# jl6017/AutoURDF

Hardware: AMD Instinct MI355X
Metric: registered frames/sec (N=4096 pts, K=20 clusters) (higher is better)
Workload: dtype f32

## Files before the change

### autourdf_amd/csrc/train_backward.hip

```cpp
#include <cmath>
#include <cstddef>
#include <cstring>
#include "train_dev.h"

namespace creg {

__device__ __forceinline__ TrainState advance_state(const TrainState& S, float loss, const Hyper& hy, double bc1, float bc2_sqrt) {
    TrainState N = S;
    const bool improved = loss < S.min_loss;
    N.last_loss = loss;
    N.epochs_run = S.epochs_run + 1;
    const int count = improved ? 0 : S.count + 1;
    N.min_loss = improved ? loss : S.min_loss;
    N.best_epoch = improved ? S.epochs_run : S.best_epoch;
    N.count = count;
    N.stopped = (!improved && count > hy.stop) ? 1 : S.stopped;
    if (!N.stopped) {
        N.step = S.step + 1;
        N.step_size = (float)(S.lr / bc1);
        N.bc2_sqrt = bc2_sqrt;
        const double cur = (double)loss;
        if (cur < S.sched_best * (1.0 - 1e-4)) { N.sched_best = cur; N.sched_bad = 0; }
        else N.sched_bad = S.sched_bad + 1;
        if (N.sched_bad > hy.patience) {
            const double nl = fmax(S.lr * (double)hy.factor, 0.0);
            if (S.lr - nl > 1e-8) N.lr = nl;
            N.sched_bad = 0;
        }
    }
    return N;
}

constexpr int GC_QMAX = 3;
__device__ __forceinline__ void gradc_role(const Dims& D, const Ws& W, int epoch, int nbx, int nby, int k) {
    __shared__ float red[4][14];
    __shared__ float s_loss;
    __shared__ float s_go[16];
    const int tid = threadIdx.x, lane = tid & 63, wv = tid >> 6;
    const TrainState S = W.state[epoch & 1];
    const int b0 = W.off[k], e0 = W.off[k + 1];
    const Hyper hy = *W.hyper;
    float a = tid < nbx ? W.lossp_x[tid] : 0.f, b = tid < nby ? W.lossp_y[tid] : 0.f;
    const float m2v = W.m2[16 * k + (tid & 15)];
    float sv[16];
#pragma unroll
    for (int i = 0; i < 16; ++i) sv[i] = W.head_save[16 * k + i];
    const float* h2cur = (epoch & 1) ? W.h2[1] : W.h2[0];
    float w3v[GC_QMAX][8], h2v[GC_QMAX];
#pragma unroll
    for (int q = 0; q < GC_QMAX; ++q) {
        const int o = min(q * 256 + tid, D.H2 - 1);
        const bool isA = o < D.HA;
        const float* Pc = (epoch & 1) ? W.P1 : W.P;
        const float* wb = isA ? Pc + D.oW3A + o : Pc + D.oW3B + (o - D.HA);
        const int stride = isA ? D.HA : D.HB, nj = isA ? D.OA : D.OB;
#pragma unroll
        for (int j = 0; j < 8; ++j) w3v[q][j] = wb[(size_t)min(j, nj - 1) * stride];
        h2v[q] = h2cur[(size_t)k * D.H2 + o];
    }
    asm volatile("" :: "v"(a), "v"(b), "v"(m2v), "v"(sv[0]), "v"(sv[1]), "v"(sv[2]), "v"(sv[3]), "v"(sv[4]), "v"(sv[5]), "v"(sv[6]), "v"(sv[7]),
                 "v"(sv[8]), "v"(sv[9]), "v"(sv[10]), "v"(sv[11]), "v"(sv[12]), "v"(sv[13]), "v"(sv[14]), "v"(sv[15]), "v"(b0), "v"(e0), "v"(hy.lr));
#pragma unroll
    for (int q = 0; q < GC_QMAX; ++q)
        asm volatile("" :: "v"(h2v[q]), "v"(w3v[q][0]), "v"(w3v[q][1]), "v"(w3v[q][2]), "v"(w3v[q][3]), "v"(w3v[q][4]), "v"(w3v[q][5]), "v"(w3v[q][6]),
                     "v"(w3v[q][7]));
    if (S.stopped) {
        if (k == 0 && tid == 0) {
            TrainState E = S; E.stopped = 1;
            W.state[(epoch + 1) & 1] = E;
        }
        return;
    }
    const int n_first = min(b0 + tid, D.NP - 1);
    const float4 p_first = W.pts4[n_first];
    const int4 c_first = W.cnt4[n_first];
    const int s_first = W.sgn_x[n_first];
    const float4 pr_first = W.pred4[n_first];
    for (int i = tid + 256; i < nbx; i += 256) a += W.lossp_x[i];
    for (int i = tid + 256; i < nby; i += 256) b += W.lossp_y[i];
    a = wave_sum_fast(a); b = wave_sum_fast(b);
    if (lane == 0) { red[wv][0] = a; red[wv][1] = b; }
    __syncthreads();
    if (tid == 0) {
        const float sa = ((red[0][0] + red[1][0]) + red[2][0]) + red[3][0];
        const float sb = ((red[0][1] + red[1][1]) + red[2][1]) + red[3][1];
        s_loss = sa / (float)D.NP + sb / (float)D.NT;
    }
    __syncthreads();
    const float loss = s_loss;
    TrainState N = advance_state(S, loss, hy, S.next_bc1, S.next_bc2s);
    const bool improved = loss < S.min_loss;
    if (improved) {
        for (int n = b0 + tid; n < e0; n += 256) {
            const float4 p = (n == b0 + tid) ? pr_first : W.pred4[n];
            W.best_pred[3 * (size_t)n] = p.x; W.best_pred[3 * (size_t)n + 1] = p.y; W.best_pred[3 * (size_t)n + 2] = p.z;
        }
        if (tid < 16) W.best_m[16 * k + tid] = m2v;
    }
    if (k == 0 && tid == 0) {
        N.next_bc1 = W.bc1[min(N.step + 1, D.epochs)];
        N.next_bc2s = W.bc2s[min(N.step + 1, D.epochs)];
        W.state[(epoch + 1) & 1] = N;
        W.loss_hist[S.epochs_run] = loss;
        W.lr_hist[S.epochs_run] = (float)S.lr;
        W.result[0] = N.min_loss; W.result[1] = (float)N.epochs_run; W.result[2] = (float)N.lr; W.result[3] = (float)N.best_epoch;
    }
    if (N.stopped) return;
    const float gx = 1.0f / (float)D.NP, gy = 1.0f / (float)D.NT;
    float acc[12];
#pragma unroll
    for (int i = 0; i < 12; ++i) acc[i] = 0.f;
    for (int n = b0 + tid; n < e0; n += 256) {
        const bool first = n == b0 + tid;
        const float4 p = first ? p_first : W.pts4[n];
        const int4 c = first ? c_first : W.cnt4[n];
        const int sb = first ? s_first : W.sgn_x[n];
        const float g[3] = {((sb & 1) ? gx : -gx) + gy * (float)c.x, ((sb & 2) ? gx : -gx) + gy * (float)c.y,
                            ((sb & 4) ? gx : -gx) + gy * (float)c.z};
#pragma unroll
        for (int q = 0; q < 3; ++q) {
            acc[4 * q] = fmaf(g[q], p.x, acc[4 * q]); acc[4 * q + 1] = fmaf(g[q], p.y, acc[4 * q + 1]);
            acc[4 * q + 2] = fmaf(g[q], p.z, acc[4 * q + 2]); acc[4 * q + 3] += g[q];
        }
    }
    __syncthreads();
#pragma unroll
    for (int i = 0; i < 12; ++i) { const float r = wave_sum_fast(acc[i]); if (lane == 0) red[wv][i] = r; }
    __syncthreads();
    if (tid == 0) {
        float G12[12];
        for (int i = 0; i < 12; ++i) G12[i] = ((red[0][i] + red[1][i]) + red[2][i]) + red[3][i];
        for (int i = 0; i < 16; ++i) W.gm2[16 * k + i] = i < 12 ? G12[i] : 0.f;
        const float G[9] = {G12[0], G12[1], G12[2], G12[4], G12[5], G12[6], G12[8], G12[9], G12[10]};
        const float gt[3] = {G12[3], G12[7], G12[11]};
        float go[16];
        for (int i = 0; i < 16; ++i) go[i] = 0.f;
        if (D.rot == ROT_6D) {
            go[0] = gt[0]; go[1] = gt[1]; go[2] = gt[2];
            rot6d_to_matrix_vjp(sv, G, go + 4);
        } else if (D.rot == ROT_RPY) {
            go[0] = gt[0]; go[1] = gt[1]; go[2] = gt[2];
            float ge[3];
            euler_xyz_to_matrix_vjp(sv, G, ge);
            for (int i = 0; i < 3; ++i) go[4 + i] = ge[i] * (1.f - sv[4 + i] * sv[4 + i]);
        } else if (D.rot == ROT_Q) {
            go[0] = gt[0]; go[1] = gt[1]; go[2] = gt[2];
            float gu[4];
            quat_to_matrix_vjp(sv, G, gu);
            const float nrm = sv[4];
            if (nrm > 1e-12f) {
                const float dot = sv[0] * gu[0] + sv[1] * gu[1] + sv[2] * gu[2] + sv[3] * gu[3];
#pragma unroll
                for (int i = 0; i < 4; ++i) go[4 + i] = (gu[i] - sv[i] * dot) / nrm;
            } else {
#pragma unroll
                for (int i = 0; i < 4; ++i) go[4 + i] = gu[i] / 1e-12f;
            }
        } else {
            float gdq[8];
            dq_to_se3_vjp(sv, G, gt, gdq);
            for (int i = 0; i < 8; ++i) go[4 + i] = gdq[i];
        }
        for (int i = 0; i < 12; ++i) { W.g_out[16 * k + i] = go[i]; s_go[i] = go[i]; }
    }
    __syncthreads();
#pragma unroll
    for (int q = 0; q < GC_QMAX; ++q) {
        const int o = q * 256 + tid;
        if (o < D.H2) {
            const bool isA = o < D.HA;
            const int nj = isA ? D.OA : D.OB, gofs = isA ? 0 : 4;
            float sum = 0.f;
#pragma unroll
            for (int j = 0; j < 8; ++j) if (j < nj) sum = fmaf(s_go[gofs + j], w3v[q][j], sum);
            W.g_h2[(size_t)k * D.H2 + o] = sum * act_grad(h2v[q], D.slope);
        }
    }
}

__global__ __launch_bounds__(256) void k_gradc(Dims D, Ws W0, int epoch, int nbx, int nby, size_t bstride) {
    asm volatile("" :: "s"(W0.P), "s"(W0.P1), "s"(W0.h2[0]), "s"(W0.h2[1]), "s"(W0.head_save), "s"(W0.m2), "s"(W0.gm2), "s"(W0.pts4), "s"(W0.pred4),
                 "s"(W0.sgn_x), "s"(W0.cnt4), "s"(W0.lossp_x), "s"(W0.lossp_y), "s"(W0.g_out), "s"(W0.g_h2), "s"(W0.state), "s"(W0.bc1), "s"(W0.bc2s),
                 "s"(W0.best_m), "s"(W0.best_pred), "s"(W0.loss_hist), "s"(W0.lr_hist), "s"(W0.result), "s"(W0.off), "s"(W0.hyper),
                 "s"(D.rot), "s"(D.K), "s"(D.H2), "s"(D.HA), "s"(D.HB), "s"(D.OA), "s"(D.OB), "s"(D.NP), "s"(D.NT), "s"(D.epochs), "s"(D.slope),
                 "s"(D.oW3A), "s"(D.oW3B), "s"(epoch), "s"(nbx), "s"(nby), "s"(bstride));
    const Ws W = ws_shift(W0, blockIdx.z * bstride);
    gradc_role(D, W, epoch, nbx, nby, blockIdx.x);
}

__device__ __forceinline__ float adam_value(float p, float& mm, float& vv, float g, float step_size, float bc2_sqrt) {
    const float b1w = (float)(1.0 - 0.9), b2 = 0.999f, b2w = (float)(1.0 - 0.999);
    mm = mm + b1w * (g - mm);
    vv = vv * b2 + (b2w * g) * g;
    const float denom = sqrtf(vv) / bc2_sqrt + 1e-8f;
    return p + (-step_size * mm) / denom;
}

#ifdef CREG_BD_STAMPS
struct BdStamps {
    unsigned long long first[256], endB[256], endD[256], startB[256], startD[256];
    unsigned long long phase[2][8], blocks[2];
    int armed;
};
__device__ BdStamps g_bd_st;
#endif
constexpr int BD_THREADS = 512;
constexpr int B2_THREADS = BD_THREADS;
constexpr int B2_WAVES = B2_THREADS / 64;
constexpr int B2_CB = 16;
constexpr int B2_RB = 32;
__host__ __device__ inline int b2_smem_floats(int K, int IN, int H2) {
    return B2_WAVES * B2_RB * B2_CB + K * IN + 2 * K * B2_CB + H2 * B2_CB;
}
__device__ __forceinline__ float row_sum16(float v) {
    CREG_DPP_STEP(v, 0xB1, 0xF);
    CREG_DPP_STEP(v, 0x4E, 0xF);
    CREG_DPP_STEP(v, 0x141, 0xF);
    CREG_DPP_STEP(v, 0x140, 0xF);
    return v;
}

template <int KW, bool X>
__device__ __forceinline__ void bwd2_role(const Dims& D, const Ws& W, int epoch, int blk, float* sh, unsigned long long bd_entry) {
    constexpr int NS = KW / 4;
    constexpr bool V4 = KW % 16 == 0;
    constexpr int NA = V4 ? NS / 4 : NS;
    float* red = sh;
    float* encs = red + B2_WAVES * B2_RB * B2_CB;
    float* gxs = encs + D.K * D.IN;
    float* xt = gxs + D.K * B2_CB;
    float* w2s = xt + D.K * B2_CB;
    const int tid = threadIdx.x, lane = tid & 63, wv = tid >> 6, lj = lane & 15, kk = lane >> 4;
    __builtin_amdgcn_s_waitcnt(0x0F70);
    const int c0 = blk * B2_CB, par = epoch & 1;
    const float* x1cur = par ? W.x1[1] : W.x1[0];
    float* x1next = par ? W.x1[0] : W.x1[1];
    const float* Pc = par ? W.P1 : W.P;
    float* Pn = par ? W.P : W.P1;
    BD_T0
    {
        const float* src = Pc + D.oW2 + (size_t)(wv * KW + (lane >> 2)) * D.H + c0 + 4 * (lane & 3);
        float* dst = w2s + wv * KW * B2_CB;
#pragma unroll
        for (int i = 0; i < KW; i += 16)
            if (i + (lane >> 2) < KW)
                __builtin_amdgcn_global_load_lds((const __attribute__((address_space(1))) void*)(src + (size_t)i * D.H),
                                                 (__attribute__((address_space(3))) void*)(dst + i * B2_CB), 16, 0, 0);
    }
    const float* gbase = W.g_h2 + wv * KW + (V4 ? 4 * kk : kk);
    auto load_a = [&](int row, float* dst) {
        const float* g = gbase + (size_t)min(row, D.K - 1) * D.H2;
#pragma unroll
        for (int q = 0; q < NA; ++q) {
            if constexpr (V4) { const float4 v = *(const float4*)(g + 16 * q); dst[4 * q] = v.x; dst[4 * q + 1] = v.y; dst[4 * q + 2] = v.z; dst[4 * q + 3] = v.w; }
            else dst[q] = g[4 * q];
        }
    };
    float a0[NS], a1[NS];
    const bool two0 = D.K > 16;
    load_a(lj, a0);
    if (two0) load_a(16 + lj, a1);
    const int half = tid >> 8, t2 = tid & 255, row = t2 >> 4, i4 = t2 & 15, hu = c0 + row;
    const bool ain = 4 * i4 < D.IN;
    const int ei = min(4 * i4, D.IN - 4);
    const size_t wi = (size_t)D.oW1 + (size_t)hu * D.IN + ei;
    float4 pw = *(const float4*)(Pc + wi), pm = *(const float4*)(W.AM + wi), pv = *(const float4*)(W.AV + wi);
    const bool ain2 = X && 64 + 4 * i4 < D.IN;
    const int ei2 = min(64 + 4 * i4, D.IN - 4);
    const size_t wi2 = (size_t)D.oW1 + (size_t)hu * D.IN + ei2;
    float4 pw2, pm2, pv2;
// ... 313 lines not shown
```

### autourdf_amd/csrc/train_dev.h

```cpp
#pragma once
#include <type_traits>
#include "creg_common.h"
#include "creg_dev.h"

namespace creg {

struct Dims {
    int rot, K, KP, IN, H, HA, HB, H2, OA, OB, NP, NT, epochs;
    float slope;
    int oW1, ob1, oW2, ob2, oW3A, ob3A, oW3B, ob3B, NPAR;
    int nbx, nby;
    int nyb;
    int npb;
    int ppl;
    int nbt, nbp;
    int rows;
};

constexpr int PS_MAXB = 512;
constexpr int YS_CHUNK = 16384;

struct Hyper {
    float lr, factor;
    int patience, stop;
};

struct TrainState {
    double lr, sched_best;
    int sched_bad, count, stopped, step;
    float min_loss;
    int epochs_run, best_epoch;
    float step_size, bc2_sqrt;
    float last_loss;
    float next_bc2s;
    double next_bc1;
};

struct Ws {
    float *P, *P1, *AM, *AV;
    float *pose_in, *enc, *x1[2], *h2[2], *head_save, *m2, *gm2;
    float4 *pts4, *y4, *pred4, *ys4, *psl4, *ps4;
    float *ybox, *pbox;
    int* sb;
    int* sgn_x;
    int4* cnt4;
    float *lossp_x, *lossp_y;
    float *g_out, *g_h2;
    TrainState* state;
    double* bc1;
    float* bc2s;
    float *best_m, *best_pred, *loss_hist, *lr_hist, *result;
    int* off;
    Hyper* hyper;
    unsigned long long* ysum;
};

static_assert(sizeof(Ws) % sizeof(char*) == 0, "Ws must hold pointers only");
__host__ __device__ __forceinline__ Ws ws_shift(Ws W, size_t bytes) {
    char** p = reinterpret_cast<char**>(&W);
#pragma unroll
    for (size_t i = 0; i < sizeof(Ws) / sizeof(char*); ++i) p[i] += bytes;
    return W;
}

constexpr int ROT_Q = 0, ROT_DQ = 1, ROT_6D = 2, ROT_RPY = 3;
constexpr int POSE_IN = 12;
typedef float f32x4 __attribute__((ext_vector_type(4)));
typedef float nn_f2 __attribute__((ext_vector_type(2)));
__device__ __forceinline__ float act_f(float v, float slope) { return v > 0.f ? v : v * slope; }
__device__ __forceinline__ float act_grad(float post, float slope) { return post > 0.f ? 1.f : slope; }

__device__ __forceinline__ int seg_of(const int* __restrict__ off, int k, int n) {
    int lo = 0, hi = k;
    while (hi - lo > 1) { const int mid = (lo + hi) >> 1; if (off[mid] <= n) lo = mid; else hi = mid; }
    return lo;
}

#ifdef CREG_BD_STAMPS
#define BD_T0 unsigned long long bd_t[8]; int bd_n = 0; if (threadIdx.x == 0) bd_t[bd_n++] = bd_entry;
#define BD_T  if (threadIdx.x == 0) bd_t[bd_n++] = wall_clock64();
#define BD_TEND(role, epoch) do { asm volatile("s_waitcnt vmcnt(0)" ::: "memory"); if (threadIdx.x == 0) { bd_t[bd_n++] = wall_clock64(); \
    if (g_bd_st.armed) { const int sl_ = (epoch) & 255; atomicMin(&g_bd_st.first[sl_], bd_t[0]); \
        atomicMin(role ? &g_bd_st.startD[sl_] : &g_bd_st.startB[sl_], bd_t[0]); atomicMax(role ? &g_bd_st.endD[sl_] : &g_bd_st.endB[sl_], bd_t[bd_n - 1]); \
        for (int k_ = 1; k_ < bd_n; ++k_) atomicAdd(&g_bd_st.phase[role][k_ - 1], bd_t[k_] - bd_t[k_ - 1]); atomicAdd(&g_bd_st.blocks[role], 1ull); } } } while (0)
#else
#define BD_T0
#define BD_T
#define BD_TEND(role, epoch)
#endif

constexpr int BATCH_MAX = 64;
struct Slice { Ws W; int nz; };

template <int V, int... Vs, typename F>
static void by_value(int v, F f) {
    if constexpr (sizeof...(Vs) == 0) f(std::integral_constant<int, V>{});
    else if (v == V) f(std::integral_constant<int, V>{});
    else by_value<Vs...>(v, f);
}
template <typename F>
static void by_nc(int H, F f) { by_value<1, 2, 4, 8>(H / 64, f); }

struct ParamMap { int off, count; };
int param_map(const Dims& D, ParamMap* pm);
constexpr int COPY_MAX = 150;
struct CopyTable { const unsigned* src[COPY_MAX]; unsigned* dst[COPY_MAX]; int n[COPY_MAX]; int count = 0; };
void copy_table_add(CopyTable& T, const void* src, void* dst, size_t bytes, hipStream_t s);
void copy_table_launch(CopyTable& T, hipStream_t s);
int setup_raise_lds(const Dims& D);
int stage_inputs(const Dims& D, const Slice& S, size_t bstride, const creg_train_args* args, hipStream_t s);
void launch_sorts(const Dims& D, const Slice& S, size_t bstride, hipStream_t s, bool keep_target_blocks);
void launch_params_home(const Dims& D, const Slice& S, size_t bstride, int sidx, int step0, hipStream_t s);
void launch_set_state(const Dims& D, const Ws& W, const creg_train_state& from, hipStream_t s);
void launch_get_state(const Ws& W, int sidx, double* out, hipStream_t s);
void launch_l2(const Dims& D, const Slice& S, size_t bstride, int par, hipStream_t s);
void launch_head(const Dims& D, const Slice& S, size_t bstride, int par, hipStream_t s);
void launch_nn(const Dims& D, const Slice& S, size_t bstride, int par, hipStream_t s);
bool backward_fits(const Dims& D);
int bd_raise_lds(const Dims& D);
void launch_gradc(const Dims& D, const Slice& S, size_t bstride, int epoch, hipStream_t s);
void launch_bd(const Dims& D, const Slice& S, size_t bstride, int epoch, hipStream_t s);
int bd_stamps_arm(bool on);

}
```

### autourdf_amd/csrc/train_engine.hip

```cpp
#include <chrono>
#include <cstdlib>
#include <cstring>
#include <memory>
#include <vector>
#include "train_dev.h"
#include "nn_l1.h"

namespace creg {

constexpr int CHAINS_MAX = 8;

struct Plan {
    creg_train_shape shape{};
    Dims D{};
    Ws W{};
    ParamMap pm[10] = {};
    int np = 0;
    int B = 1;
    size_t bstride = 0;
    int branches = 1;
    hipGraphExec_t gexec = nullptr;
    bool graph_ready = false;
    int graph_epochs = 0;
    bool chain_streams = false;
// ... 176 lines not shown

static int pick_chain_streams(Plan* P, hipStream_t s) {
    static const bool probe = !(getenv("CREG_NO_QUEUE_PROBE") && getenv("CREG_NO_QUEUE_PROBE")[0] == '1');
    constexpr int ATTEMPTS = 7;
    P->probe_us = 0;
    auto fits = [](double t) { return t >= 0 && t < SPIN_TOGETHER_US; };
    auto accept = [&](double t) { if (P->probe_us >= 0 && (int)t > P->probe_us) P->probe_us = (int)t; };
    for (int gi = 1; gi < P->branches; ++gi) {
        hipStream_t set[CHAINS_MAX + 1], rejected[ATTEMPTS + 1];
        int ns = 0, nr = 0;
        set[ns++] = s;
        for (int j = 1; j < gi; ++j) set[ns++] = P->cst[j];
        hipStream_t chosen = nullptr;
        if (P->cst[gi]) {
            set[ns] = P->cst[gi];
            const double t = candidate_spin_us(set, ns + 1);
            if (!probe || fits(t)) { chosen = P->cst[gi]; if (probe) accept(t); }
            else { (void)hipStreamSynchronize(P->cst[gi]); rejected[nr++] = P->cst[gi]; P->cst[gi] = nullptr; }
        }
        for (int attempt = 0; !chosen && attempt < ATTEMPTS; ++attempt) {
            hipStream_t cs = nullptr;
            if (hipStreamCreateWithFlags(&cs, hipStreamNonBlocking) != hipSuccess) break;
            if (!probe) { chosen = cs; break; }
            set[ns] = cs;
            const double t = candidate_spin_us(set, ns + 1);
            if (fits(t)) { chosen = cs; accept(t); }
            else rejected[nr++] = cs;
        }
        if (!chosen && nr) { chosen = rejected[--nr]; P->probe_us = -1; }
        for (int i = 0; i < nr; ++i) (void)hipStreamDestroy(rejected[i]);
        if (!chosen) {
            (void)hipGetLastError();
            creg::set_error("creg_train_plan_run_batch: cannot create a stream for chain %d", gi);
            return CREG_EHIP;
        }
        P->cst[gi] = chosen;
    }
    P->cal_stream = s; P->cal_done = true;
    return CREG_OK;
}

static int capture_chains(Plan* P, int epg) {
    FirstError fe;
    if (!P->cfork) CREG_TRY(fe, hipEventCreateWithFlags(&P->cfork, hipEventDisableTiming));
    ScopedStream cs;
    CREG_TRY(fe, hipStreamCreateWithFlags(&cs.h, hipStreamNonBlocking));
    for (int gi = 0; gi < P->branches && fe.ok(); ++gi) {
        ScopedGraph g;
        if (gi > 0 && !P->cjoin[gi]) CREG_TRY(fe, hipEventCreateWithFlags(&P->cjoin[gi], hipEventDisableTiming));
        if (P->cexec[gi]) { (void)hipGraphExecDestroy(P->cexec[gi]); P->cexec[gi] = nullptr; }
        CREG_TRY(fe, hipStreamBeginCapture(cs.h, hipStreamCaptureModeThreadLocal));
        if (fe.ok()) {
            const Slice S = chain_slice(P, gi);
            for (int i = 0; i < epg; ++i) enqueue_epoch(P, S, i, cs.h);
            fe.note(hipStreamEndCapture(cs.h, &g.h), "hipStreamEndCapture");
        }
        CREG_TRY(fe, hipGraphInstantiate(&P->cexec[gi], g.h, nullptr, nullptr, 0));
    }
    if (!fe.ok()) {
        (void)hipGetLastError();
        for (int gi = 0; gi < CHAINS_MAX; ++gi) if (P->cexec[gi]) { (void)hipGraphExecDestroy(P->cexec[gi]); P->cexec[gi] = nullptr; }
        creg::set_error("creg_train_plan_run_batch: chain graph capture failed: %s: %s", fe.what, hipGetErrorString(fe.err));
        return CREG_EHIP;
    }
    P->graph_ready = true;
    P->graph_epochs = epg;
    return CREG_OK;
}

static int run_chains(Plan* P, hipStream_t s) {
    const Dims& D = P->D;
    if (P->branches > 1 && (!P->cal_done || P->cal_stream != s))
        if (int rc = pick_chain_streams(P, s)) return rc;
    auto st_of = [&](int gi) { return gi == 0 ? s : P->cst[gi]; };
    FirstError fe;
    CREG_TRY(fe, hipEventRecord(P->cfork, s));
    for (int gi = 1; gi < P->branches; ++gi) CREG_TRY(fe, hipStreamWaitEvent(P->cst[gi], P->cfork, 0));
    int e = 0;
    for (; fe.ok() && e + P->graph_epochs <= D.epochs; e += P->graph_epochs)
        for (int gi = 0; gi < P->branches; ++gi) CREG_TRY(fe, hipGraphLaunch(P->cexec[gi], st_of(gi)));
    for (int gi = 0; fe.ok() && gi < P->branches; ++gi) {
        const Slice S = chain_slice(P, gi);
        for (int e2 = e; e2 < D.epochs; ++e2) enqueue_epoch(P, S, e2, st_of(gi));
    }
    for (int gi = 1; gi < P->branches; ++gi) {
        if (hipEventRecord(P->cjoin[gi], P->cst[gi]) != hipSuccess || hipStreamWaitEvent(s, P->cjoin[gi], 0) != hipSuccess) {
            (void)hipStreamSynchronize(P->cst[gi]);
            fe.note(hipErrorUnknown, "joining a chain stream");
        }
    }
    if (!fe.ok()) {
        (void)hipGetLastError();
        creg::set_error("creg_train_plan_run_batch: %s: %s", fe.what, hipGetErrorString(fe.err));
        return CREG_EHIP;
    }
    return CREG_OK;
}

static int begin_run(const char* who, Plan* P, const Slice& S, const creg_train_args* args, bool with_outputs, bool may_keep_leaves,
                     hipStream_t s) {
    bool keep = may_keep_leaves && P->target_blocks_valid;
    for (int b = 0; b < S.nz; ++b) {
        const creg_train_args* a = args + b;
        CREG_REQUIRE(a->m && a->y && a->local_pts && a->seg_offsets && a->params && (!with_outputs || (a->best_m && a->best_pred && a->result)),
                     "%s: null pointer in problem %d", who, b);
        for (int i = 0; i < P->np; ++i) CREG_REQUIRE(a->params[i], "%s: params[%d] of problem %d is null", who, i, b);
        keep = keep && a->y_unchanged != 0;
    }
    if (int rc = stage_inputs(P->D, S, P->bstride, args, s)) return rc;
    launch_sorts(P->D, S, P->bstride, s, keep);
    P->target_blocks_valid = may_keep_leaves;
    return CREG_OK;
}

static void results_out(const Plan* P, const Slice& S, const creg_train_args* args, CopyTable& T, hipStream_t s) {
    const Dims& D = P->D;
    for (int b = 0; b < S.nz; ++b) {
        const creg_train_args* a = args + b;
        const Ws W = ws_shift(S.W, (size_t)b * P->bstride);
        for (int i = 0; i < P->np; ++i) copy_table_add(T, W.P + P->pm[i].off, a->params[i], sizeof(float) * P->pm[i].count, s);
        copy_table_add(T, W.best_m, a->best_m, sizeof(float) * 16 * D.K, s);
        copy_table_add(T, W.best_pred, a->best_pred, sizeof(float) * 3 * D.NP, s);
        copy_table_add(T, W.result, a->result, sizeof(float) * 4, s);
        if (a->loss_hist) copy_table_add(T, W.loss_hist, a->loss_hist, sizeof(float) * D.epochs, s);
        if (a->lr_hist) copy_table_add(T, W.lr_hist, a->lr_hist, sizeof(float) * D.epochs, s);
    }
    copy_table_launch(T, s);
}

static int batch_of(const creg_train_shape* s) { return s->batch >= 1 ? s->batch : 1; }

extern "C" size_t creg_train_workspace_bytes(const creg_train_shape* shape) {
    Dims D;
    if (!make_dims(shape, &D) || shape->batch < 0 || shape->batch > BATCH_MAX) return 0;
    return align_up(carve(D, nullptr, nullptr), 256) * batch_of(shape);
}

extern "C" int creg_train_plan_create(const creg_train_shape* shape, void* workspace, size_t workspace_bytes,
                                      creg_train_plan** plan) {
    Dims D;
    CREG_REQUIRE(plan && workspace, "creg_train_plan_create: null pointer");
    CREG_REQUIRE(make_dims(shape, &D), "creg_train_plan_create: unsupported shape (rot in 0..3, hidden in {64, 128, 256, 512}, 1 <= k <= 256 with the K x IN features + the B role's tiles inside 160 KB of LDS, sizes >= 1)");
    CREG_REQUIRE(((uintptr_t)workspace & 255) == 0, "creg_train_plan_create: workspace must be 256-byte aligned");
    CREG_REQUIRE(shape->batch >= 0 && shape->batch <= BATCH_MAX, "creg_train_plan_create: batch must be in [0, %d]", BATCH_MAX);
    const size_t one = align_up(carve(D, nullptr, nullptr), 256), need = one * batch_of(shape);
    CREG_REQUIRE(workspace_bytes >= need, "creg_train_plan_create: workspace too small (%zu < %zu)", workspace_bytes, need);
    auto P = std::make_unique<Plan>();
    P->shape = *shape; P->D = D; P->np = param_map(D, P->pm);
    carve(D, (char*)workspace, &P->W);
    P->B = batch_of(shape); P->bstride = one;
    const int auto_chains = (D.NT > 64 * 64 && P->B >= 3) ? 3 : (P->B >= 8 ? 3 : (P->B >= 5 ? 2 : 1));
    P->chain_streams = shape->graph_branches <= 0;
    P->branches = shape->graph_branches > 0 ? shape->graph_branches : (shape->graph_branches < 0 ? -shape->graph_branches : auto_chains);
    if (P->branches > P->B) P->branches = P->B;
    if (P->branches > CHAINS_MAX) P->branches = CHAINS_MAX;
    if (int rc = bd_raise_lds(D)) return rc;
    if (int rc = setup_raise_lds(D)) return rc;
    *plan = (creg_train_plan*)P.release();
    return CREG_OK;
}

extern "C" int creg_train_plan_run_batch(creg_train_plan* plan, const creg_train_args* args, int32_t n,
                                         creg_stream_t stream) {
    Plan* P = (Plan*)plan;
    CREG_REQUIRE(P && args, "creg_train_plan_run_batch: null pointer");
    CREG_REQUIRE(n == P->B, "creg_train_plan_run_batch: the plan was created for a batch of %d problems, got %d", P->B, n);
    hipStream_t s = (hipStream_t)stream;
    const Dims& D = P->D;
    const Slice all = slice_of(P, 0, P->B);
    if (int rc = begin_run("creg_train_plan_run_batch", P, all, args, true, true, s)) return rc;
    int e = 0;
    if (P->shape.use_graph && D.epochs >= 2) {
        int epg = P->shape.use_graph > 1 ? P->shape.use_graph : 50;
        if (epg > D.epochs) epg = D.epochs;
        epg &= ~1;
        if (!P->graph_ready) {
            const int rc = P->chain_streams ? capture_chains(P, epg) : capture_epochs(P, epg);
            if (rc) return rc;
        }
        if (P->chain_streams) {
            if (int rc = run_chains(P, s)) { P->target_blocks_valid = false; return rc; }
            e = D.epochs;
        } else {
            for (; e + P->graph_epochs <= D.epochs; e += P->graph_epochs) CREG_HIP(hipGraphLaunch(P->gexec, s));
        }
    }
    for (; e < D.epochs; ++e) enqueue_epoch(P, all, e, s);
    launch_params_home(D, all, P->bstride, D.epochs & 1, 0, s);
    CREG_LAUNCH_CHECK();
    CopyTable T;
    results_out(P, all, args, T, s);
    return CREG_OK;
}

extern "C" int creg_train_plan_run(creg_train_plan* plan, const creg_train_args* a, creg_stream_t stream) {
    return creg_train_plan_run_batch(plan, a, 1, stream);
}

extern "C" int creg_train_plan_resume(creg_train_plan* plan, const creg_train_args* a, const creg_train_state* from, int32_t n_epochs,
                                      float* const* exp_avg_out, float* const* exp_avg_sq_out, double* state_out, creg_stream_t stream) {
    Plan* P = (Plan*)plan;
    CREG_REQUIRE(P && a && from, "creg_train_plan_resume: null pointer");
    CREG_REQUIRE(from->exp_avg && from->exp_avg_sq, "creg_train_plan_resume: the state needs both Adam moment arrays");
    const Dims& D = P->D;
    CREG_REQUIRE(n_epochs >= 1 && from->step >= 0 && from->epochs_run >= 0 && from->step + n_epochs <= D.epochs && from->epochs_run + n_epochs <= D.epochs,
                 "creg_train_plan_resume: step %d / epochs_run %d + %d epochs exceed the plan's %d", from->step, from->epochs_run, n_epochs, D.epochs);
    CREG_REQUIRE(from->lr >= 0.0 && from->sched_bad >= 0 && from->count >= 0, "creg_train_plan_resume: negative lr or counter");
    const ParamMap* pm = P->pm;
    const int np = P->np;
    for (int i = 0; i < np; ++i) CREG_REQUIRE(from->exp_avg[i] && from->exp_avg_sq[i], "creg_train_plan_resume: moment tensor %d is null", i);
    hipStream_t s = (hipStream_t)stream;
    const Slice one = slice_of(P, 0, 1);
    if (int rc = begin_run("creg_train_plan_resume", P, one, a, true, false, s)) return rc;
    CopyTable T;
    for (int i = 0; i < np; ++i) {
        copy_table_add(T, from->exp_avg[i], P->W.AM + pm[i].off, sizeof(float) * pm[i].count, s);
        copy_table_add(T, from->exp_avg_sq[i], P->W.AV + pm[i].off, sizeof(float) * pm[i].count, s);
    }
    if (from->best_epoch >= 0) {
        copy_table_add(T, a->best_m, P->W.best_m, sizeof(float) * 16 * D.K, s);
        copy_table_add(T, a->best_pred, P->W.best_pred, sizeof(float) * 3 * D.NP, s);
    }
    copy_table_launch(T, s);
    launch_set_state(D, P->W, *from, s);
    for (int e = 0; e < n_epochs; ++e) enqueue_epoch(P, one, e, s);
    launch_params_home(D, one, P->bstride, n_epochs & 1, from->step, s);
    if (state_out) launch_get_state(P->W, n_epochs & 1, state_out, s);
    CREG_LAUNCH_CHECK();
    for (int i = 0; i < np; ++i) {
        if (exp_avg_out && exp_avg_out[i]) copy_table_add(T, P->W.AM + pm[i].off, exp_avg_out[i], sizeof(float) * pm[i].count, s);
        if (exp_avg_sq_out && exp_avg_sq_out[i]) copy_table_add(T, P->W.AV + pm[i].off, exp_avg_sq_out[i], sizeof(float) * pm[i].count, s);
    }
    results_out(P, one, a, T, s);
    CREG_LAUNCH_CHECK();
    return CREG_OK;
}

extern "C" int creg_train_plan_probe(creg_train_plan* plan, const creg_train_args* a, float* m2, float* pred,
                                     float* loss, float* grad_m2, creg_stream_t stream) {
    Plan* P = (Plan*)plan;
    CREG_REQUIRE(P && a, "creg_train_plan_probe: null pointer");
    hipStream_t s = (hipStream_t)stream;
    const Dims& D = P->D; const Ws& W = P->W;
    const Slice one = slice_of(P, 0, 1);
    if (int rc = begin_run("creg_train_plan_probe", P, one, a, false, false, s)) return rc;
    launch_head(D, one, P->bstride, 0, s);
    launch_nn(D, one, 0, 0, s);
    launch_gradc(D, one, 0, 0, s);
    CREG_LAUNCH_CHECK();
    if (m2) CREG_HIP(hipMemcpyAsync(m2, W.m2, sizeof(float) * 16 * D.K, hipMemcpyDeviceToDevice, s));
    if (pred) CREG_HIP(hipMemcpyAsync(pred, W.best_pred, sizeof(float) * 3 * D.NP, hipMemcpyDeviceToDevice, s));
    if (loss) CREG_HIP(hipMemcpyAsync(loss, W.loss_hist, sizeof(float), hipMemcpyDeviceToDevice, s));
    if (grad_m2) CREG_HIP(hipMemcpyAsync(grad_m2, W.gm2, sizeof(float) * 16 * D.K, hipMemcpyDeviceToDevice, s));
    return CREG_OK;
}

extern "C" int creg_train_plan_profile(creg_train_plan* plan, const creg_train_args* a, int32_t n_epochs,
                                       float* us_out, creg_stream_t stream) {
    Plan* P = (Plan*)plan;
    CREG_REQUIRE(P && a && us_out && n_epochs >= 1, "creg_train_plan_profile: bad argument");
    hipStream_t s = (hipStream_t)stream;
    const int br = P->shape.use_graph ? P->branches : 1;
    const int nzb = P->B / br + (P->B % br ? 1 : 0);
    std::vector<creg_train_args> all((size_t)nzb, *a);
    const Slice S = slice_of(P, 0, nzb);
    if (int rc = begin_run("creg_train_plan_profile", P, S, all.data(), false, false, s)) return rc;
    ScopedEvents ev((size_t)(NKERN + 1) * n_epochs);
    for (auto& e : ev.v) CREG_HIP(hipEventCreate(&e));
    for (int e = 0; e < n_epochs; ++e) enqueue_epoch(P, S, e, s, ev.v.data() + (NKERN + 1) * e);
    CREG_LAUNCH_CHECK();
    CREG_HIP(hipStreamSynchronize(s));
    double acc[NKERN] = {0};
    for (int e = 0; e < n_epochs; ++e)
        for (int k = 0; k < NKERN; ++k) {
            float ms = 0.f;
            CREG_HIP(hipEventElapsedTime(&ms, ev[(NKERN + 1) * e + k], ev[(NKERN + 1) * e + k + 1]));
            acc[k] += ms;
        }
    us_out[0] = 0.f;
    for (int k = 0; k < NKERN; ++k) us_out[1 + k] = (float)(acc[k] * 1000.0 / n_epochs);
    const int REP = 200;
    const Dims& D = P->D;
    auto b2b = [&](auto launch, float* out) -> int {
        float ms = 0.f;
        CREG_HIP(hipEventRecord(ev[0], s));
        for (int i = 0; i < REP; ++i) launch(i);
        CREG_HIP(hipEventRecord(ev[1], s));
        CREG_HIP(hipStreamSynchronize(s));
        CREG_HIP(hipEventElapsedTime(&ms, ev[0], ev[1]));
        *out = ms * 1000.f / REP;
        return CREG_OK;
    };
    if (int rc = b2b([&](int) { launch_nn(D, S, P->bstride, 0, s); }, us_out + 6)) return rc;
    us_out[7] = (float)S.nz;
    if (int rc = bd_stamps_arm(true)) return rc;
    if (int rc = b2b([&](int i) { launch_bd(D, S, P->bstride, i, s); }, us_out + 8)) return rc;
    if (int rc = bd_stamps_arm(false)) return rc;
    if (int rc = b2b([&](int i) { launch_l2(D, S, P->bstride, i & 1, s); }, us_out + 9)) return rc;
    if (int rc = b2b([&](int i) { launch_head(D, S, P->bstride, i & 1, s); }, us_out + 10)) return rc;
    if (int rc = b2b([&](int i) { launch_gradc(D, S, P->bstride, i, s); }, us_out + 11)) return rc;
    CREG_LAUNCH_CHECK();
    return CREG_OK;
}

extern "C" int creg_train_plan_info(const creg_train_plan* plan, creg_train_plan_info_t* info) {
    CREG_REQUIRE(plan && info, "creg_train_plan_info: null pointer");
    const Plan* P = (const Plan*)plan;
    info->pruned_target_search = P->D.rows ? 2 : (P->D.nyb > 0);
    info->pruned_predicted_search = P->D.npb > 0;
    info->graph_branches = P->branches;
    info->batch = P->B;
    info->epochs_per_graph = P->shape.use_graph ? P->graph_epochs : 0;
    info->nn_points_per_lane = P->D.ppl;
    info->nn_boxes_target = P->D.nbt;
    info->nn_boxes_predicted = P->D.nbp;
    info->chain_probe_us = P->probe_us;
    return CREG_OK;
}

extern "C" int creg_train_plan_destroy(creg_train_plan* plan) {
    delete (Plan*)plan;
    return CREG_OK;
}
```

### autourdf_amd/csrc/train_setup.hip

```cpp
#include <cfloat>
#include <cmath>
#include <cstring>
#include "train_dev.h"

namespace creg {

constexpr int PREP_MAXB = 64;
static_assert(PREP_MAXB == BATCH_MAX, "k_prep's tables hold a whole batch");
struct PrepBatch { const float* m[PREP_MAXB]; const float* y[PREP_MAXB]; const float* pts[PREP_MAXB]; Hyper hy[PREP_MAXB]; };
__global__ __launch_bounds__(256) void k_prep(Dims D, Ws W0, size_t bstride, PrepBatch pb) {
    const Ws W = ws_shift(W0, blockIdx.z * bstride);
    const Hyper hy = pb.hy[blockIdx.z];
    const float* __restrict__ m = pb.m[blockIdx.z];
    const float* __restrict__ y = pb.y[blockIdx.z];
    const float* __restrict__ pts = pb.pts[blockIdx.z];
    const int t = blockIdx.x * 256 + threadIdx.x;
    const int stride = gridDim.x * 256;
    for (int n = t; n < D.NP; n += stride) {
        const int c = seg_of(W.off, D.K, n);
        W.pts4[n] = make_float4(pts[3 * (size_t)n], pts[3 * (size_t)n + 1], pts[3 * (size_t)n + 2], __int_as_float(c));
    }
    for (int j = t; j < D.NT; j += stride)
        W.y4[j] = make_float4(y[3 * (size_t)j], y[3 * (size_t)j + 1], y[3 * (size_t)j + 2], 0.f);
    for (int i = t; i < D.NPAR; i += stride) { W.AM[i] = 0.f; W.AV[i] = 0.f; }
    for (int i = t; i < D.epochs; i += stride) { W.loss_hist[i] = NAN; W.lr_hist[i] = NAN; }
    for (int i = t; i < (D.KP - D.K) * D.H; i += stride) { W.x1[0][D.K * D.H + i] = 0.f; W.x1[1][D.K * D.H + i] = 0.f; }
    for (int i = t; i < (D.KP - D.K) * D.H2; i += stride) { W.h2[0][D.K * D.H2 + i] = 0.f; W.h2[1][D.K * D.H2 + i] = 0.f; W.g_h2[D.K * D.H2 + i] = 0.f; }
    for (int i = t; i < (D.KP - D.K) * 16; i += stride) W.g_out[D.K * 16 + i] = 0.f;
    for (int i = t; i <= D.epochs; i += stride) { W.bc1[i] = 1.0 - pow(0.9, (double)i); W.bc2s[i] = (float)sqrt(1.0 - pow(0.999, (double)i)); }
    if (blockIdx.x == 0) {
        for (int r = threadIdx.x; r < D.K; r += 256) {
            const float* M = m + 16 * r;
            const float R[9] = {M[0], M[1], M[2], M[4], M[5], M[6], M[8], M[9], M[10]};
            const float tr[3] = {M[3], M[7], M[11]};
            float in[POSE_IN];
            for (int i = 0; i < POSE_IN; ++i) in[i] = 0.f;
            int nin;
            if (D.rot == ROT_Q) {
                float q[4];
                matrix_to_quat(R, q);
                in[0] = tr[0]; in[1] = tr[1]; in[2] = tr[2]; in[3] = q[0]; in[4] = q[1]; in[5] = q[2]; in[6] = q[3];
                nin = 7;
            } else if (D.rot == ROT_DQ) {
                se3_to_dq(R, tr, in, FLT_EPSILON);
                nin = 8;
            } else if (D.rot == ROT_6D) {
                in[0] = tr[0]; in[1] = tr[1]; in[2] = tr[2];
                for (int i = 0; i < 6; ++i) in[3 + i] = R[i];
                nin = 9;
            } else {
                in[0] = tr[0]; in[1] = tr[1]; in[2] = tr[2];
                matrix_to_euler_xyz(R, in + 3);
                nin = 6;
            }
            for (int i = 0; i < POSE_IN; ++i) W.pose_in[POSE_IN * r + i] = in[i];
            float* e = W.enc + (size_t)r * D.IN;
            for (int f = 0; f < 4; ++f) {
                const float mul = (float)(1 << f);
                for (int i = 0; i < nin; ++i) {
                    e[(2 * f) * nin + i] = sinf(mul * in[i]);
                    e[(2 * f + 1) * nin + i] = cosf(mul * in[i]);
                }
            }
        }
        if (threadIdx.x == 0) {
            TrainState s;
            *W.hyper = hy;
            s.lr = (double)hy.lr; s.sched_best = INFINITY; s.sched_bad = 0; s.count = 0; s.stopped = 0;
            s.step = 0; s.min_loss = 1000.f; s.epochs_run = 0; s.best_epoch = -1; s.step_size = 0.f;
            s.bc2_sqrt = 1.f; s.last_loss = NAN;
            s.next_bc1 = 1.0 - 0.9; s.next_bc2s = (float)sqrt(1.0 - 0.999);
            W.state[0] = s; W.state[1] = s;
        }
    }
}

__global__ __launch_bounds__(256) void k_l1(Dims D, Ws W0, int par, size_t bstride) {
    const Ws W = ws_shift(W0, blockIdx.z * bstride);
    const int lane = threadIdx.x & 63;
    const int o = blockIdx.x * 4 + (threadIdx.x >> 6);
    if (o >= D.H) return;
    const float w = lane < D.IN ? W.P[D.oW1 + (size_t)o * D.IN + lane] : 0.f;
    const float w2 = 64 + lane < D.IN ? W.P[D.oW1 + (size_t)o * D.IN + 64 + lane] : 0.f;
    const float b = W.P[D.ob1 + o];
    for (int r = 0; r < D.K; ++r) {
        float t = lane < D.IN ? w * W.enc[(size_t)r * D.IN + lane] : 0.f;
        if (64 + lane < D.IN) t = fmaf(w2, W.enc[(size_t)r * D.IN + 64 + lane], t);
        const float v = wave_sum_fast(t) + b;
        if (lane == 0) (par ? W.x1[1] : W.x1[0])[(size_t)r * D.H + o] = act_f(v, D.slope);
    }
}

__device__ __forceinline__ unsigned ordered_bits(float c) {
    unsigned u = (unsigned)__float_as_int(c);
    u = (u & 0x80000000u) ? ~u : (u | 0x80000000u);
    return u == 0xFFFFFFFFu ? 0xFFFFFFFEu : u;
}
__device__ __forceinline__ void bitonic_segments(unsigned long long* key, int npow, int seg, int tid, int nthreads) {
    bool wide_before = true;
    for (int size = 2; size <= seg; size <<= 1)
        for (int stride = size >> 1; stride >= 1; stride >>= 1) {
            const bool wide = stride > 64;
            if (wide || wide_before) __syncthreads();
            else { __builtin_amdgcn_fence(__ATOMIC_SEQ_CST, "wavefront"); __builtin_amdgcn_wave_barrier(); }
            for (int t = tid; t < (npow >> 1); t += nthreads) {
                const int i = ((t & ~(stride - 1)) << 1) | (t & (stride - 1)), j = i | stride;
                const unsigned long long a = key[i], b = key[j];
                const bool up = size == seg || (i & size) == 0;
                if ((a > b) == up) { key[i] = b; key[j] = a; }
            }
            wide_before = wide;
        }
    __syncthreads();
}
static int pow2_at_least(int n) { int p = 64; while (p < n) p <<= 1; return p; }

__global__ __launch_bounds__(1024) void k_sort_y(Dims D, Ws W0, size_t bstride, int npow, int check) {
    const Ws W = ws_shift(W0, blockIdx.z * bstride);
    extern __shared__ __attribute__((aligned(16))) char smem_raw[];
    unsigned long long* key = (unsigned long long*)smem_raw;
    const int tid = threadIdx.x, lane = tid & 63, wv = tid >> 6;
    const int BS = 64 * D.ppl;
    const int base = blockIdx.x * YS_CHUNK, nc = min(YS_CHUNK, D.NT - base);
    const int blk0 = base / BS, nblk = (nc + BS - 1) / BS;
    __shared__ unsigned long long s_fp;
    {
        if (tid == 0) s_fp = 0ull;
        __syncthreads();
        unsigned long long h = 0ull;
        for (int j = tid; j < nc; j += 1024) {
            const float4 p = W.y4[base + j];
            const unsigned long long a = (unsigned)__float_as_int(p.x), b = (unsigned)__float_as_int(p.y), c = (unsigned)__float_as_int(p.z);
            unsigned long long v = a ^ (b << 21) ^ (c << 42) ^ (c >> 22);
            v *= 0x9E3779B97F4A7C15ull;
            h += (v ^ (v >> 29)) * (2ull * (unsigned long long)j + 1ull);
        }
        atomicAdd(&s_fp, h);
        __syncthreads();
        const unsigned long long fp = s_fp ^ ((unsigned long long)nc << 48) ^ (unsigned long long)D.ppl ^ ((unsigned long long)D.rows << 8);
        if (check && W.ysum[blockIdx.x] == fp) return;
        __syncthreads();
        if (tid == 0) W.ysum[blockIdx.x] = fp;
    }
    for (int j = tid; j < npow; j += 1024) key[j] = j < nc ? (unsigned long long)j : ~0ull;
    __syncthreads();
    int level = 0;
    for (int seg = npow; seg > (D.rows ? 16 : BS); seg >>= 1, ++level) {
        const int axis = level % 3;
        for (int j = tid; j < npow; j += 1024) {
            const unsigned long long k = key[j];
            if (k != ~0ull) {
                const int idx = (int)(k & 0xFFFFull);
                const float4 p = W.y4[base + idx];
// ... 59 lines not shown
    int npow = 64;
    while (npow < ns) npow <<= 1;
    if (npow > YS_CHUNK) {
        for (int sl = tid; sl < ns; sl += 512) {
            float4 o = make_float4(0.f, 0.f, 0.f, __int_as_float(0x7fffffff));
            if (sl < n) { const float4 p = W.pts4[p0 + sl]; o = make_float4(p.x, p.y, p.z, __int_as_float(p0 + sl)); }
            W.psl4[(size_t)first * BS + sl] = o;
        }
        return;
    }
    for (int sl = tid; sl < npow; sl += 512) key[sl] = sl >= ns ? ~0ull : sl < n ? (unsigned long long)(p0 + sl) : 0xFFFFull;
    for (int b = tid; b < m; b += 512) { sf[b] = 0; sm[b] = (unsigned short)m; }
    __syncthreads();
    int levels = 0;
    for (int level = 0; level < 9; ++level) {
        if (tid == 0) s_more = 0;
        __syncthreads();
        for (int b = tid; b < m; b += 512) if (sm[b] > 1) s_more = 1;
        __syncthreads();
        if (!s_more) break;
        levels = level + 1;
        const int axis = level % 3;
        for (int sl = tid; sl < ns; sl += 512) {
            const unsigned idx = (unsigned)(key[sl] & 0xFFFFull);
            unsigned u = 0xFFFFFFFFu;
            if (idx != 0xFFFFu) {
                const float4 p = W.pts4[idx];
                u = ordered_bits(axis == 0 ? p.x : axis == 1 ? p.y : p.z);
            }
            key[sl] = ((unsigned long long)sf[sl >> bshift] << 48) | ((unsigned long long)u << 16) | idx;
        }
        __syncthreads();
        bitonic_segments(key, npow, npow, tid, 512);
        unsigned short nf = 0, nm = 0;
        const bool mine = tid < m;
        if (mine) {
            const int f = sf[tid], mm = sm[tid];
            nf = (unsigned short)f; nm = (unsigned short)mm;
            if (mm >= 2) {
                const int ml = mm >> 1;
                if (tid < f + ml) nm = (unsigned short)ml;
                else { nf = (unsigned short)(f + ml); nm = (unsigned short)(mm - ml); }
            }
        }
        __syncthreads();
        if (mine) { sf[tid] = nf; sm[tid] = nm; }
        __syncthreads();
    }
    if (D.rows)
        for (int sub = 0; sub < 2; ++sub) {
            const int axis = (levels + sub) % 3;
            __syncthreads();
            for (int sl = tid; sl < ns; sl += 512) {
                const unsigned idx = (unsigned)(key[sl] & 0xFFFFull);
                unsigned u = 0xFFFFFFFFu;
                if (idx != 0xFFFFu) {
                    const float4 p = W.pts4[idx];
                    u = ordered_bits(axis == 0 ? p.x : axis == 1 ? p.y : p.z);
                }
                key[sl] = ((unsigned long long)u << 16) | idx;
            }
            __syncthreads();
            bitonic_segments(key, npow, 64 >> sub, tid, 512);
        }
    for (int sl = tid; sl < ns; sl += 512) {
        const unsigned idx = (unsigned)(key[sl] & 0xFFFFull);
        float4 o = make_float4(0.f, 0.f, 0.f, __int_as_float(0x7fffffff));
        if (idx != 0xFFFFu) { const float4 p = W.pts4[idx]; o = make_float4(p.x, p.y, p.z, __int_as_float((int)idx)); }
        W.psl4[(size_t)first * BS + sl] = o;
    }
}

__global__ __launch_bounds__(256) void k_params_home(Dims D, Ws W0, size_t bstride, int sidx, int step0) {
    const Ws W = ws_shift(W0, blockIdx.z * bstride);
    if (((W.state[sidx].step - step0) & 1) == 0) return;
    for (int i = blockIdx.x * 256 + threadIdx.x; i < D.NPAR; i += gridDim.x * 256) W.P[i] = W.P1[i];
}

struct ResumeState { double lr, sched_best; int step, epochs_run, sched_bad, count, best_epoch, stopped; float min_loss; };
__global__ void k_set_state(Dims D, Ws W, ResumeState rs) {
    if (threadIdx.x || blockIdx.x) return;
    TrainState s = W.state[0];
    s.lr = rs.lr; s.sched_best = rs.sched_best; s.sched_bad = rs.sched_bad; s.count = rs.count; s.stopped = rs.stopped; s.step = rs.step;
    s.min_loss = rs.min_loss; s.epochs_run = rs.epochs_run; s.best_epoch = rs.best_epoch;
    s.next_bc1 = W.bc1[min(rs.step + 1, D.epochs)]; s.next_bc2s = W.bc2s[min(rs.step + 1, D.epochs)];
    W.state[0] = s; W.state[1] = s;
    W.result[0] = s.min_loss; W.result[1] = (float)s.epochs_run; W.result[2] = (float)s.lr; W.result[3] = (float)s.best_epoch;
}
__global__ void k_get_state(Ws W, int sidx, double* out) {
    if (threadIdx.x || blockIdx.x) return;
    const TrainState s = W.state[sidx];
    out[0] = s.step; out[1] = s.epochs_run; out[2] = s.lr; out[3] = s.sched_best; out[4] = s.sched_bad; out[5] = s.count;
    out[6] = (double)s.min_loss; out[7] = s.best_epoch; out[8] = s.stopped; out[9] = (double)s.last_loss; out[10] = 0.0; out[11] = 0.0;
}

__global__ __launch_bounds__(256) void k_copy_table(CopyTable T) {
    const unsigned* __restrict__ s = T.src[blockIdx.y]; unsigned* __restrict__ d = T.dst[blockIdx.y];
    const int n = T.n[blockIdx.y];
    for (int i = blockIdx.x * 256 + threadIdx.x; i < n; i += gridDim.x * 256) d[i] = s[i];
}
void copy_table_launch(CopyTable& T, hipStream_t s) {
    if (T.count) hipLaunchKernelGGL(k_copy_table, dim3(32, T.count), dim3(256), 0, s, T);
    T.count = 0;
}
void copy_table_add(CopyTable& T, const void* src, void* dst, size_t bytes, hipStream_t s) {
    if (T.count == COPY_MAX) copy_table_launch(T, s);
    T.src[T.count] = (const unsigned*)src; T.dst[T.count] = (unsigned*)dst; T.n[T.count] = (int)(bytes / 4); ++T.count;
}

int param_map(const Dims& D, ParamMap* pm) {
    if (D.rot != ROT_DQ) {
        const ParamMap m[10] = {{D.oW1, D.H * D.IN}, {D.ob1, D.H}, {D.oW2, D.HA * D.H}, {D.ob2, D.HA},
                                {D.oW3A, D.OA * D.HA}, {D.ob3A, D.OA}, {D.oW2 + D.HA * D.H, D.HB * D.H},
                                {D.ob2 + D.HA, D.HB}, {D.oW3B, D.OB * D.HB}, {D.ob3B, D.OB}};
        memcpy(pm, m, sizeof(m));
        return 10;
    }
    const ParamMap m[6] = {{D.oW1, D.H * D.IN}, {D.ob1, D.H}, {D.oW2, D.HB * D.H}, {D.ob2, D.HB}, {D.oW3B, D.OB * D.HB}, {D.ob3B, D.OB}};
    memcpy(pm, m, sizeof(m));
    return 6;
}

static int ys_sort_npow(const Dims& D) { return pow2_at_least(D.NT < YS_CHUNK ? D.NT : YS_CHUNK); }
static int ys_sort_smem(const Dims& D) {
    const int per_chunk = YS_CHUNK / (64 * D.ppl);
    return ys_sort_npow(D) * 8 + 6 * 4 * (D.nyb < per_chunk ? D.nyb : per_chunk) * D.ppl;
}
static int ps_sort_smem(const Dims& D) {
    const int BS = 64 * D.ppl;
    const int np = pow2_at_least((D.NP + BS - 1) / BS * BS);
    return (np < YS_CHUNK ? np : YS_CHUNK) * 8;
}
constexpr int YS_SORT_LDS_MAX = YS_CHUNK * 8 + 6 * 4 * (YS_CHUNK / 64), PS_SORT_LDS_MAX = YS_CHUNK * 8;
int setup_raise_lds(const Dims& D) {
    if (D.npb) CREG_HIP(hipFuncSetAttribute((const void*)k_sort_p, hipFuncAttributeMaxDynamicSharedMemorySize, PS_SORT_LDS_MAX));
    if (D.nyb) CREG_HIP(hipFuncSetAttribute((const void*)k_sort_y, hipFuncAttributeMaxDynamicSharedMemorySize, YS_SORT_LDS_MAX));
    return CREG_OK;
}
void launch_sorts(const Dims& D, const Slice& S, size_t bstride, hipStream_t s, bool keep_target_blocks) {
    if (D.nyb) hipLaunchKernelGGL(k_sort_y, dim3(cdiv(D.NT, YS_CHUNK), 1, S.nz), dim3(1024), ys_sort_smem(D), s, D, S.W, bstride, ys_sort_npow(D), keep_target_blocks ? 1 : 0);
    if (D.npb) hipLaunchKernelGGL(k_sort_p, dim3(D.K, 1, S.nz), dim3(512), ps_sort_smem(D), s, D, S.W, bstride);
}

int stage_inputs(const Dims& D, const Slice& S, size_t bstride, const creg_train_args* args, hipStream_t s) {
    const int n = S.nz;
    ParamMap pm[10];
    const int np = param_map(D, pm);
    CopyTable T;
    PrepBatch pb;
    for (int b = 0; b < n; ++b) {
        const creg_train_args* a = args + b;
        const Ws W = ws_shift(S.W, (size_t)b * bstride);
        for (int i = 0; i < np; ++i) copy_table_add(T, a->params[i], W.P + pm[i].off, sizeof(float) * pm[i].count, s);
        copy_table_add(T, a->seg_offsets, W.off, sizeof(int) * (D.K + 1), s);
        pb.m[b] = a->m; pb.y[b] = a->y; pb.pts[b] = a->local_pts;
        pb.hy[b] = Hyper{a->lr, a->sched_factor, a->sched_patience, a->stop};
    }
    copy_table_launch(T, s);
    const int mx = D.NP > D.NT ? D.NP : D.NT;
    int blocks = cdiv(mx > D.NPAR ? mx : D.NPAR, 256);
    if (blocks > 2048) blocks = 2048;
    hipLaunchKernelGGL(k_prep, dim3(blocks, 1, n), dim3(256), 0, s, D, S.W, bstride, pb);
    hipLaunchKernelGGL(k_l1, dim3(cdiv(D.H, 4), 1, n), dim3(256), 0, s, D, S.W, 0, bstride);
    launch_l2(D, S, bstride, 0, s);
    CREG_LAUNCH_CHECK();
    return CREG_OK;
}
// ... 12 lines not shown
```

Baseline: 164.9.

## Defer best-prediction cloud write to a single post-training kernel

Stops the gradient kernel from copying the predicted point cloud to best_pred on every improving epoch. It now only saves the best per-cluster transform, and after the epoch loop a new kernel rebuilds best_pred from the points and that transform. An 'improved' flag is added to the training state, in former padding, so the rebuild is skipped when no epoch improved. This removes repeated global stores and the pred4 load from the hot epoch kernel. The cost is one extra launch per fit and a dependence on best_m reproducing the same prediction.

```diff
diff --git a/autourdf_amd/csrc/train_backward.hip b/autourdf_amd/csrc/train_backward.hip
--- a/autourdf_amd/csrc/train_backward.hip
+++ b/autourdf_amd/csrc/train_backward.hip
@@ -13,6 +13,7 @@
     const int count = improved ? 0 : S.count + 1;
     N.min_loss = improved ? loss : S.min_loss;
     N.best_epoch = improved ? S.epochs_run : S.best_epoch;
+    N.improved = improved ? 1 : S.improved;
     N.count = count;
     N.stopped = (!improved && count > hy.stop) ? 1 : S.stopped;
     if (!N.stopped) {
@@ -75,7 +76,6 @@
     const float4 p_first = W.pts4[n_first];
     const int4 c_first = W.cnt4[n_first];
     const int s_first = W.sgn_x[n_first];
-    const float4 pr_first = W.pred4[n_first];
     for (int i = tid + 256; i < nbx; i += 256) a += W.lossp_x[i];
     for (int i = tid + 256; i < nby; i += 256) b += W.lossp_y[i];
     a = wave_sum_fast(a); b = wave_sum_fast(b);
@@ -90,13 +90,7 @@
     const float loss = s_loss;
     TrainState N = advance_state(S, loss, hy, S.next_bc1, S.next_bc2s);
     const bool improved = loss < S.min_loss;
-    if (improved) {
-        for (int n = b0 + tid; n < e0; n += 256) {
-            const float4 p = (n == b0 + tid) ? pr_first : W.pred4[n];
-            W.best_pred[3 * (size_t)n] = p.x; W.best_pred[3 * (size_t)n + 1] = p.y; W.best_pred[3 * (size_t)n + 2] = p.z;
-        }
-        if (tid < 16) W.best_m[16 * k + tid] = m2v;
-    }
+    if (improved && tid < 16) W.best_m[16 * k + tid] = m2v;
     if (k == 0 && tid == 0) {
         N.next_bc1 = W.bc1[min(N.step + 1, D.epochs)];
         N.next_bc2s = W.bc2s[min(N.step + 1, D.epochs)];
@@ -179,13 +173,30 @@
 }
 
 __global__ __launch_bounds__(256) void k_gradc(Dims D, Ws W0, int epoch, int nbx, int nby, size_t bstride) {
-    asm volatile("" :: "s"(W0.P), "s"(W0.P1), "s"(W0.h2[0]), "s"(W0.h2[1]), "s"(W0.head_save), "s"(W0.m2), "s"(W0.gm2), "s"(W0.pts4), "s"(W0.pred4),
+    asm volatile("" :: "s"(W0.P), "s"(W0.P1), "s"(W0.h2[0]), "s"(W0.h2[1]), "s"(W0.head_save), "s"(W0.m2), "s"(W0.gm2), "s"(W0.pts4),
                  "s"(W0.sgn_x), "s"(W0.cnt4), "s"(W0.lossp_x), "s"(W0.lossp_y), "s"(W0.g_out), "s"(W0.g_h2), "s"(W0.state), "s"(W0.bc1), "s"(W0.bc2s),
-                 "s"(W0.best_m), "s"(W0.best_pred), "s"(W0.loss_hist), "s"(W0.lr_hist), "s"(W0.result), "s"(W0.off), "s"(W0.hyper),
+                 "s"(W0.best_m), "s"(W0.loss_hist), "s"(W0.lr_hist), "s"(W0.result), "s"(W0.off), "s"(W0.hyper),
                  "s"(D.rot), "s"(D.K), "s"(D.H2), "s"(D.HA), "s"(D.HB), "s"(D.OA), "s"(D.OB), "s"(D.NP), "s"(D.NT), "s"(D.epochs), "s"(D.slope),
                  "s"(D.oW3A), "s"(D.oW3B), "s"(epoch), "s"(nbx), "s"(nby), "s"(bstride));
     const Ws W = ws_shift(W0, blockIdx.z * bstride);
     gradc_role(D, W, epoch, nbx, nby, blockIdx.x);
+}
+
+__global__ __launch_bounds__(256) void k_best_cloud(Dims D, Ws W0, int sidx, size_t bstride) {
+    const Ws W = ws_shift(W0, blockIdx.z * bstride);
+    const int k = blockIdx.x, b0 = max(W.off[k], 0), e0 = min(W.off[k + 1], D.NP);
+    if (!W.state[sidx].improved) return;
+    float m[12];
+#pragma unroll
+    for (int i = 0; i < 12; ++i) m[i] = W.best_m[16 * k + i];
+    for (int n = b0 + (int)threadIdx.x; n < e0; n += 256) {
+        const float4 p = W.pts4[n];
+#pragma unroll
+        for (int a = 0; a < 3; ++a) W.best_pred[3 * (size_t)n + a] = fmaf(p.z, m[4 * a + 2], fmaf(p.y, m[4 * a + 1], p.x * m[4 * a])) + m[4 * a + 3];
+    }
+}
+void launch_best_cloud(const Dims& D, const Slice& S, size_t bstride, int sidx, hipStream_t s) {
+    hipLaunchKernelGGL(k_best_cloud, dim3(D.K, 1, S.nz), dim3(256), 0, s, D, S.W, sidx, bstride);
 }
 
 __device__ __forceinline__ float adam_value(float p, float& mm, float& vv, float g, float step_size, float bc2_sqrt) {
diff --git a/autourdf_amd/csrc/train_dev.h b/autourdf_amd/csrc/train_dev.h
--- a/autourdf_amd/csrc/train_dev.h
+++ b/autourdf_amd/csrc/train_dev.h
@@ -33,6 +33,7 @@
     float step_size, bc2_sqrt;
     float last_loss;
     float next_bc2s;
+    int improved;
     double next_bc1;
 };
 
@@ -55,6 +56,7 @@
     unsigned long long* ysum;
 };
 
+static_assert(sizeof(TrainState) == 72, "`improved` sits in what was padding: the state stays nine 8-byte words");
 static_assert(sizeof(Ws) % sizeof(char*) == 0, "Ws must hold pointers only");
 __host__ __device__ __forceinline__ Ws ws_shift(Ws W, size_t bytes) {
     char** p = reinterpret_cast<char**>(&W);
@@ -120,6 +122,7 @@
 int bd_raise_lds(const Dims& D);
 void launch_gradc(const Dims& D, const Slice& S, size_t bstride, int epoch, hipStream_t s);
 void launch_bd(const Dims& D, const Slice& S, size_t bstride, int epoch, hipStream_t s);
+void launch_best_cloud(const Dims& D, const Slice& S, size_t bstride, int sidx, hipStream_t s);
 int bd_stamps_arm(bool on);
 
 }
diff --git a/autourdf_amd/csrc/train_engine.hip b/autourdf_amd/csrc/train_engine.hip
--- a/autourdf_amd/csrc/train_engine.hip
+++ b/autourdf_amd/csrc/train_engine.hip
@@ -282,6 +282,7 @@
     for (int gi = 0; fe.ok() && gi < P->branches; ++gi) {
         const Slice S = chain_slice(P, gi);
         for (int e2 = e; e2 < D.epochs; ++e2) enqueue_epoch(P, S, e2, st_of(gi));
+        launch_best_cloud(D, S, P->bstride, D.epochs & 1, st_of(gi));
     }
     for (int gi = 1; gi < P->branches; ++gi) {
         if (hipEventRecord(P->cjoin[gi], P->cst[gi]) != hipSuccess || hipStreamWaitEvent(s, P->cjoin[gi], 0) != hipSuccess) {
@@ -385,7 +386,9 @@
             for (; e + P->graph_epochs <= D.epochs; e += P->graph_epochs) CREG_HIP(hipGraphLaunch(P->gexec, s));
         }
     }
+    const bool chains_ran = P->shape.use_graph && D.epochs >= 2 && P->chain_streams;
     for (; e < D.epochs; ++e) enqueue_epoch(P, all, e, s);
+    if (!chains_ran) launch_best_cloud(D, all, P->bstride, D.epochs & 1, s);
     launch_params_home(D, all, P->bstride, D.epochs & 1, 0, s);
     CREG_LAUNCH_CHECK();
     CopyTable T;
@@ -424,6 +427,7 @@
     copy_table_launch(T, s);
     launch_set_state(D, P->W, *from, s);
     for (int e = 0; e < n_epochs; ++e) enqueue_epoch(P, one, e, s);
+    launch_best_cloud(D, one, P->bstride, n_epochs & 1, s);
     launch_params_home(D, one, P->bstride, n_epochs & 1, from->step, s);
     if (state_out) launch_get_state(P->W, n_epochs & 1, state_out, s);
     CREG_LAUNCH_CHECK();
@@ -447,6 +451,7 @@
     launch_head(D, one, P->bstride, 0, s);
     launch_nn(D, one, 0, 0, s);
     launch_gradc(D, one, 0, 0, s);
+    launch_best_cloud(D, one, 0, 1, s);
     CREG_LAUNCH_CHECK();
     if (m2) CREG_HIP(hipMemcpyAsync(m2, W.m2, sizeof(float) * 16 * D.K, hipMemcpyDeviceToDevice, s));
     if (pred) CREG_HIP(hipMemcpyAsync(pred, W.best_pred, sizeof(float) * 3 * D.NP, hipMemcpyDeviceToDevice, s));
diff --git a/autourdf_amd/csrc/train_setup.hip b/autourdf_amd/csrc/train_setup.hip
--- a/autourdf_amd/csrc/train_setup.hip
+++ b/autourdf_amd/csrc/train_setup.hip
@@ -68,7 +68,7 @@
             *W.hyper = hy;
             s.lr = (double)hy.lr; s.sched_best = INFINITY; s.sched_bad = 0; s.count = 0; s.stopped = 0;
             s.step = 0; s.min_loss = 1000.f; s.epochs_run = 0; s.best_epoch = -1; s.step_size = 0.f;
-            s.bc2_sqrt = 1.f; s.last_loss = NAN;
+            s.bc2_sqrt = 1.f; s.last_loss = NAN; s.improved = 0;
             s.next_bc1 = 1.0 - 0.9; s.next_bc2s = (float)sqrt(1.0 - 0.999);
             W.state[0] = s; W.state[1] = s;
         }
@@ -294,7 +294,7 @@
     if (threadIdx.x || blockIdx.x) return;
     TrainState s = W.state[0];
     s.lr = rs.lr; s.sched_best = rs.sched_best; s.sched_bad = rs.sched_bad; s.count = rs.count; s.stopped = rs.stopped; s.step = rs.step;
-    s.min_loss = rs.min_loss; s.epochs_run = rs.epochs_run; s.best_epoch = rs.best_epoch;
+    s.min_loss = rs.min_loss; s.epochs_run = rs.epochs_run; s.best_epoch = rs.best_epoch; s.improved = 0;
     s.next_bc1 = W.bc1[min(rs.step + 1, D.epochs)]; s.next_bc2s = W.bc2s[min(rs.step + 1, D.epochs)];
     W.state[0] = s; W.state[1] = s;
     W.result[0] = s.min_loss; W.result[1] = (float)s.epochs_run; W.result[2] = (float)s.lr; W.result[3] = (float)s.best_epoch;
```

Result: slower. 162.5 (-1.5%).
